# dohlee/diffab-pytorch

Hardware: AMD Instinct MI355X
Metric: CDR-residue denoise-steps/sec (K=128 patch) (higher is better)
Workload: dtype f32 (bf16x6 / fp16x3 split-precision products on the 16-bit matrix cores, fp32 accumulate; fp32-accurate, DESIGN section 4)

## Files before the change

diffab-pytorch_amd/csrc/ipa_persistent.hip:

```cpp
#include "common.h"
#include "denoiser_internal.h"
#define AT_STAMP_REALTIME 1
#include "ipa_attn_tile.h"
#include "proj_frames_h3_tile.h"
#include "rowgemm_h3_tile.h"
#include "mlp_chain_tile.h"

namespace diffab {

namespace {
constexpr size_t cmax(size_t a, size_t b) { return a > b ? a : b; }
constexpr size_t kModuleLdsBytes = cmax(cmax(ipa_attn_lds_bytes(8), static_cast<size_t>(kChainLdsBytes)),
                                        cmax(static_cast<size_t>(pjh3::PJ_LDS_BYTES), static_cast<size_t>(h3tile::lds_bytes<128>())));

struct ModuleArgs {
  float* xa;
  float* xb;
  float* proj;
  float* feat;
  const float* pair;
  const float* esc;
  const int* ctx_of_row;
  const float* R;
  const float* t;
  const char* planes;
  size_t layer_stride, pj_off, out_off, wis_off, small_off;
  unsigned long long* stamps;
  const float* emb_X;
  MlpChainSet emb, heads;
  int B, NL;
  int stagger_ticks, stagger_classes;
};
}

template <int KRES>
__global__ __launch_bounds__(512) void ipa_module_persistent_kernel(const ModuleArgs a) {
  extern __shared__ __attribute__((aligned(16))) float lds[];
  constexpr int K = KRES, NTILE = K / TI, DT = K / 128;
  static_assert(KRES == 128 || KRES == 256, "patch-resident module: K = 128 or 256");
  const int M = a.B * K;
  if (a.stagger_ticks > 0 && a.stagger_classes > 1) {
    const unsigned long long t0 = __builtin_amdgcn_s_memrealtime();
    const unsigned long long wait = static_cast<unsigned long long>((blockIdx.x >> 3) % a.stagger_classes) * a.stagger_ticks;
    while (__builtin_amdgcn_s_memrealtime() - t0 < wait) __builtin_amdgcn_s_sleep(32);
  }
  unsigned long long* pstamps = a.stamps ? a.stamps + static_cast<size_t>(a.B) * a.NL * NTILE * 64 : nullptr;
  auto pstamp = [&](int b, int l, int k) {
    if (pstamps != nullptr && threadIdx.x == 0) pstamps[(static_cast<size_t>(b) * a.NL + l) * 4 + k] = __builtin_amdgcn_s_memrealtime();
  };
#pragma unroll 1
  for (int b = blockIdx.x; b < a.B; b += gridDim.x) {
    if (a.emb_X != nullptr) {
#pragma unroll 1
      for (int dt = 0; dt < DT; ++dt) {
        int tid = threadIdx.x;
        asm volatile("" : "+v"(tid));
        chaintile::mlp_chain_tile(reinterpret_cast<__bf16*>(lds), tid, b * DT + dt, a.emb_X, 128, a.emb.c[0].planes[0], a.emb.c[0].planes[1],
                                  nullptr, a.emb.c[0].bias[0], a.emb.c[0].bias[1], nullptr, a.emb.c[0].bias_idx0, a.emb.c[0].bias_div0, 2, 128,
                                  a.xa, 128, M);
        asm volatile("s_waitcnt vmcnt(0)" ::: "memory");
        __syncthreads();
      }
    }
#pragma unroll 1
    for (int l = 0; l < a.NL; ++l) {
      const char* lp = a.planes + static_cast<size_t>(l) * a.layer_stride;
      const float* small = reinterpret_cast<const float*>(lp + a.small_off);
      const float* xin = (l & 1) ? a.xb : a.xa;
      float* xout = (l & 1) ? a.xa : a.xb;
      pstamp(b, l, 0);
#pragma unroll 1
      for (int dt = 0; dt < DT; ++dt) {
        int tid = threadIdx.x;
        asm volatile("" : "+v"(tid));
        pjh3::proj_frames_h3_tile<true, false>(reinterpret_cast<_Float16*>(lds), tid, b * DT + dt, 0, 1, xin,
                                               reinterpret_cast<const _Float16*>(lp + a.pj_off), reinterpret_cast<const float*>(lp + a.wis_off),
                                               a.R, a.t, a.proj, M);
        if (dt + 1 < DT) {
          asm volatile("s_waitcnt vmcnt(0)" ::: "memory");
          __syncthreads();
        }
      }
      asm volatile("s_waitcnt vmcnt(0)" ::: "memory");
      __syncthreads();
      pstamp(b, l, 1);
#pragma unroll 1
      for (int tile = 0; tile < NTILE; ++tile) {
        ipa_attn_tile<8, (KRES > 128), true>(lds, b, tile, static_cast<unsigned>((b * a.NL + l) * NTILE + tile), a.proj, a.pair, a.R, a.t, small,
                                             small + 512, a.feat, K / 128, a.stamps, a.esc, nullptr, nullptr, a.ctx_of_row);
        asm volatile("s_waitcnt vmcnt(0)" ::: "memory");
        __syncthreads();
      }
      pstamp(b, l, 2);
#pragma unroll 1
      for (int dt = 0; dt < DT; ++dt) {
        int tid = threadIdx.x;
        asm volatile("" : "+v"(tid));
        h3tile::rowgemm128_h3_tile<false, 128>(reinterpret_cast<_Float16*>(lds), tid, b * DT + dt, a.feat, AF,
                                               reinterpret_cast<const _Float16*>(lp + a.out_off),
                                               reinterpret_cast<const float*>(lp + a.wis_off) + ANP, small + 576, nullptr, 0, xout, 128, M, AF);
        if (dt + 1 < DT) {
          asm volatile("s_waitcnt vmcnt(0)" ::: "memory");
          __syncthreads();
        }
      }
      asm volatile("s_waitcnt vmcnt(0)" ::: "memory");
      __syncthreads();
      pstamp(b, l, 3);
    }
    if (a.emb_X != nullptr) {
      const float* xfin = (a.NL & 1) ? a.xb : a.xa;
#pragma unroll 1
      for (int hdt = 0; hdt < 3 * DT; ++hdt) {
        const int hd = hdt / DT, dt = hdt % DT;
        int tid = threadIdx.x;
        asm volatile("" : "+v"(tid));
#define HSEL(f) (hd == 0 ? a.heads.c[0].f : hd == 1 ? a.heads.c[1].f : a.heads.c[2].f)
        chaintile::mlp_chain_tile(reinterpret_cast<__bf16*>(lds), tid, b * DT + dt, xfin, 128, HSEL(planes[0]), HSEL(planes[1]), HSEL(planes[2]),
                                  HSEL(bias[0]), HSEL(bias[1]), HSEL(bias[2]), HSEL(bias_idx0), HSEL(bias_div0), 3, HSEL(n_out),
                                  hd == 0 ? a.heads.Y[0] : hd == 1 ? a.heads.Y[1] : a.heads.Y[2],
                                  hd == 0 ? a.heads.ldy[0] : hd == 1 ? a.heads.ldy[1] : a.heads.ldy[2], M);
#undef HSEL
        asm volatile("s_waitcnt vmcnt(0)" ::: "memory");
        __syncthreads();
      }
    }
  }
}

namespace {
int g_stagger_ticks = 1000, g_stagger_classes = 8;
unsigned long long* g_module_stamps = nullptr;
}
void set_module_stagger(int ticks, int classes) {
  g_stagger_ticks = ticks;
  g_stagger_classes = classes;
}
void set_module_stamps(void* p) { g_module_stamps = static_cast<unsigned long long*>(p); }

bool ipa_module_persistent_supported(const diffab_dims* d) {
  return fast_path_supported(d) && (d->K == 128 || d->K == 256) && d->NL >= 1;
}

int launch_ipa_module_persistent(const diffab_dims* d, float* xa, float* xb, const float* R, const float* t, float* ws, const void* planes,
                                 const float* pair_planes, hipStream_t st, const float* emb_X, const MlpChainSet* emb,
                                 const MlpChainSet* heads, const int* ctx_of_row, int n_ctx) {
  DIFFAB_REQUIRE(ipa_module_persistent_supported(d) && xa && xb && R && t && ws && planes && pair_planes, DIFFAB_ERR_ARG,
                 "ipa_module_persistent: unsupported operands");
  const size_t rows = static_cast<size_t>(d->B) * d->K;
  ModuleArgs a{};
  a.xa = xa;
  a.xb = xb;
  a.proj = ws;
  a.feat = ws + rows * ANP;
  a.pair = pair_planes + 64;
  a.esc = pair_row_scales(d, pair_planes, n_ctx);
  a.ctx_of_row = ctx_of_row;
  a.R = R;
  a.t = t;
  a.planes = static_cast<const char*>(planes);
  a.layer_stride = ipa_layer_planes_bytes();
  a.pj_off = ipa_layer_h3_pj_offset();
  a.out_off = ipa_layer_h3_out_offset();
  a.wis_off = ipa_layer_h3_wis_offset();
  a.small_off = ipa_layer_small_offset();
  a.stamps = g_module_stamps;
  if (emb_X != nullptr) {
    DIFFAB_REQUIRE(emb && heads && d->D == 128 && (reinterpret_cast<uintptr_t>(emb_X) & 15) == 0, DIFFAB_ERR_ARG,
                   "ipa_module_persistent: the fused MLP phases need both chain sets");
    a.emb_X = emb_X;
    a.emb = *emb;
    a.heads = *heads;
  }
  a.B = d->B;
  a.NL = d->NL;
  a.stagger_ticks = g_stagger_ticks;
  a.stagger_classes = g_stagger_classes;
  int dev = 0, ncu = 256;
  if (hipGetDevice(&dev) == hipSuccess) (void)hipDeviceGetAttribute(&ncu, hipDeviceAttributeMultiprocessorCount, dev);
  const int grid = d->B < ncu ? d->B : ncu;
#define MODULE_LAUNCH(K_)                                                                                                       \
  do {                                                                                                                            \
    DIFFAB_HIP_CHECK(hipFuncSetAttribute(reinterpret_cast<const void*>(ipa_module_persistent_kernel<K_>),                         \
                                         hipFuncAttributeMaxDynamicSharedMemorySize, static_cast<int>(kModuleLdsBytes)));        \
    timer_begin(st);                                                                                                              \
    hipLaunchKernelGGL((ipa_module_persistent_kernel<K_>), dim3(grid), dim3(512), kModuleLdsBytes, st, a);                        \
    timer_end(st);                                                                                                                \
  } while (0)
  if (d->K == 128) MODULE_LAUNCH(128);
  else MODULE_LAUNCH(256);
#undef MODULE_LAUNCH
  DIFFAB_LAUNCH_CHECK();
  return DIFFAB_OK;
}

}
```

diffab-pytorch_amd/csrc/proj_frames_h3_tile.h:

```cpp
#pragma once
#include <hip/hip_runtime.h>
#include <cstdint>

#include "rowgemm_h3_tile.h"

namespace diffab {
namespace pjh3 {
using h3tile::f16x8;
using h3tile::f32x4;
using h3tile::h3_scale;
using h3tile::split2;
#define PJH3_FENCE() asm volatile("" ::: "memory")
constexpr int PJ_NP = 1344, PJ_GQ = 768;
constexpr int PJ_B = 96, PJ_NB = PJ_NP / PJ_B, PJ_ROWS = 128;
constexpr int PJ_LD = 80;
constexpr int PJ_STAGE_ELEMS = 2 * PJ_B * 64;
constexpr int PJ_STAGE_LDS = 2 * PJ_B * PJ_LD;
constexpr int PJ_LDS_BYTES = 2 * PJ_STAGE_LDS * 2 + PJ_ROWS * 12 * 4 + PJ_ROWS * 4;
struct __attribute__((packed, aligned(4))) pj_f3 { float x, y, z; };
__device__ __forceinline__ float mul1(float a, float b) {
#pragma clang fp contract(off)
  return a * b;
}

template <bool FULL, bool SPLIT = false, bool PROJ = true>
__device__ __forceinline__ void proj_frames_h3_tile(_Float16* __restrict__ pj_lds, const int tid, const int tile_m, const int split_i,
                                                    const int split_n, const float* __restrict__ X, const _Float16* __restrict__ Wc,
                                                    const float* __restrict__ wis, const float* __restrict__ R, const float* __restrict__ t,
                                                    float* __restrict__ Y, int M, const int nb_rt = 0, const int n_rt = 0, const int ldy_rt = 0) {
  const int NB = PROJ ? PJ_NB : nb_rt, ldy = PROJ ? PJ_NP : ldy_rt, frames_from = PROJ ? PJ_GQ / PJ_B : NB;
  const int blk0 = SPLIT ? (NB * split_i) / split_n : 0;
  const int blk1 = SPLIT ? (NB * (split_i + 1)) / split_n : NB;
  float* Rt = reinterpret_cast<float*>(pj_lds + 2 * PJ_STAGE_LDS);
  float* Sx = Rt + PJ_ROWS * 12;
  const int lane = tid & 63, wv = tid >> 6;
  const int l15 = lane & 15, g = lane >> 4, rw = wv & 3, cw = wv >> 2;
  const int m0 = tile_m * PJ_ROWS;
  float* ybase = Y + static_cast<int64_t>(m0 + 32 * rw + 4 * g) * ldy + 48 * cw + 3 * l15;
  const int col0 = 48 * cw + 3 * l15;

  int st_dst[3];
#pragma unroll
  for (int i = 0; i < 3; ++i) {
    const int idx = tid + 512 * i, pl = idx / 768, rem = idx % 768;
    st_dst[i] = (pl * PJ_B + (rem >> 3)) * PJ_LD + (rem & 7) * 8;
  }
  f32x4 wreg[3];
  const int NSTAGE = 2 * blk1;
  auto load_w = [&](int stg) {
    stg = stg < NSTAGE ? stg : NSTAGE - 1;
    const _Float16* src = Wc + static_cast<size_t>(stg) * PJ_STAGE_ELEMS + tid * 8;
#pragma unroll
    for (int i = 0; i < 3; ++i) wreg[i] = *reinterpret_cast<const f32x4*>(src + 512 * 8 * i);
  };
  auto store_w = [&](int buf) {
#pragma unroll
    for (int i = 0; i < 3; ++i) *reinterpret_cast<f32x4*>(pj_lds + buf * PJ_STAGE_LDS + st_dst[i]) = wreg[i];
  };
  load_w(2 * blk0);
  f16x8 a[2][4][2];
#pragma unroll
  for (int mt = 0; mt < 2; ++mt) {
    const int row = m0 + 32 * rw + 16 * mt + l15;
    f32x4 v[4][2];
    float m = 0.0f;
#pragma unroll
    for (int q = 0; q < 4; ++q) {
      v[q][0] = v[q][1] = f32x4{0.f, 0.f, 0.f, 0.f};
      if (FULL || row < M) {
        const float* xp = X + static_cast<int64_t>(row) * 128 + 32 * q + 8 * g;
        v[q][0] = *reinterpret_cast<const f32x4*>(xp);
        v[q][1] = *reinterpret_cast<const f32x4*>(xp + 4);
      }
#pragma unroll
      for (int c = 0; c < 8; ++c) m = fmaxf(m, fabsf(v[q][c >> 2][c & 3]));
    }
    m = fmaxf(m, __shfl_xor(m, 16));
    m = fmaxf(m, __shfl_xor(m, 32));
    float s, is;
    h3_scale(m, s, is);
    if (g == 0) Sx[32 * rw + 16 * mt + l15] = is;
#pragma unroll
    for (int q = 0; q < 4; ++q)
#pragma unroll
      for (int c = 0; c < 8; ++c) {
        _Float16 h1, h2;
        split2(v[q][c >> 2][c & 3] * s, h1, h2);
        a[mt][q][0][c] = h1;
        a[mt][q][1][c] = h2;
      }
  }
  for (int idx = tid; PROJ && idx < PJ_ROWS * 12; idx += 512) {
    const int row = idx / 12, cc = idx % 12, gr = m0 + row;
    float v = 0.0f;
    if (FULL || gr < M) v = cc < 9 ? R[static_cast<int64_t>(gr) * 9 + cc] : t[static_cast<int64_t>(gr) * 3 + (cc - 9)];
    Rt[idx] = v;
  }
  PJH3_FENCE();
  store_w(0);
  load_w(2 * blk0 + 1);
  PJH3_FENCE();
  __syncthreads();

  auto epilogue_piece = [&](const f32x4 (&acc)[2][3], const pj_f3 wsc, int blk, int piece) {
    const int mt = piece >> 2, r = piece & 3;
    const int lrow = 32 * rw + 16 * mt + 4 * g + r;
    const float isx = Sx[lrow];
    const float vx = mul1(acc[mt][0][r], mul1(isx, wsc.x)), vy = mul1(acc[mt][1][r], mul1(isx, wsc.y)), vz0 = mul1(acc[mt][2][r], mul1(isx, wsc.z));
    float ox = vx, oy = vy, oz = vz0;
    if (PROJ && blk >= frames_from) {
      const f32x4* F = reinterpret_cast<const f32x4*>(Rt + lrow * 12);
      const f32x4 f0 = F[0], f1 = F[1], f2 = F[2];
      const float vz = vz0;
      ox = __builtin_fmaf(vz, f1[2], __builtin_fmaf(vy, f0[3], mul1(vx, f0[0]))) + f2[1];
      oy = __builtin_fmaf(vz, f1[3], __builtin_fmaf(vy, f1[0], mul1(vx, f0[1]))) + f2[2];
      oz = __builtin_fmaf(vz, f2[0], __builtin_fmaf(vy, f1[1], mul1(vx, f0[2]))) + f2[3];
    }
    if (FULL || m0 + lrow < M) {
      float* yp = ybase + (16 * mt + r) * ldy + PJ_B * blk;
      if constexpr (PROJ) {
        pj_f3 o{ox, oy, oz};
        *reinterpret_cast<pj_f3*>(yp) = o;
      } else {
        const int c = PJ_B * blk + col0;
        if (c < n_rt) yp[0] = ox;
        if (c + 1 < n_rt) yp[1] = oy;
        if (c + 2 < n_rt) yp[2] = oz;
      }
    }
  };
  auto run_block = [&](f32x4 (&cur)[2][3], const f32x4 (&prev)[2][3], const pj_f3 wprev, int blk) {
#pragma unroll
    for (int mt = 0; mt < 2; ++mt)
#pragma unroll
      for (int tt = 0; tt < 3; ++tt) cur[mt][tt] = f32x4{0.f, 0.f, 0.f, 0.f};
#pragma unroll
    for (int kh = 0; kh < 2; ++kh) {
      store_w(kh ^ 1);
      load_w(2 * blk + kh + 2);
      PJH3_FENCE();
      const _Float16* wl = pj_lds + kh * PJ_STAGE_LDS + (48 * cw + l15) * PJ_LD + 8 * g;
#pragma unroll
      for (int ks = 0; ks < 2; ++ks) {
        f16x8 b[3][2];
#pragma unroll
        for (int pl = 0; pl < 2; ++pl)
#pragma unroll
          for (int tt = 0; tt < 3; ++tt) b[tt][pl] = *reinterpret_cast<const f16x8*>(wl + (pl * PJ_B + 16 * tt) * PJ_LD + 32 * ks);
#pragma unroll
        for (int term = 0; term < 3; ++term) {
          const int pa = term == 0 ? 1 : 0, pb = term == 1 ? 1 : 0;
#pragma unroll
          for (int mt = 0; mt < 2; ++mt)
#pragma unroll
            for (int tt = 0; tt < 3; ++tt)
              cur[mt][tt] = __builtin_amdgcn_mfma_f32_16x16x32_f16(a[mt][2 * kh + ks][pa], b[tt][pb], cur[mt][tt], 0, 0, 0);
          if (kh == 0 && blk > blk0) {
            epilogue_piece(prev, wprev, blk - 1, 4 * ks + term);
            if (term == 2) epilogue_piece(prev, wprev, blk - 1, 4 * ks + 3);
            __builtin_amdgcn_sched_barrier(0);
          }
        }
      }
      __syncthreads();
    }
  };
  auto wsc_of = [&](int blk) { return *reinterpret_cast<const pj_f3*>(wis + PJ_B * blk + col0); };
  f32x4 accA[2][3], accB[2][3];
  pj_f3 wA = wsc_of(blk0), wB = wA;
  int blk = blk0;
  for (; blk + 1 < blk1; blk += 2) {
    run_block(accA, accB, wB, blk);
    wB = wsc_of(blk + 1);
    run_block(accB, accA, wA, blk + 1);
    if (blk + 2 < blk1) wA = wsc_of(blk + 2);
  }
  if ((SPLIT || !PROJ) && blk < blk1) {
    run_block(accA, accB, wB, blk);
#pragma unroll
    for (int piece = 0; piece < 8; ++piece) epilogue_piece(accA, wA, blk, piece);
  } else {
#pragma unroll
    for (int piece = 0; piece < 8; ++piece) epilogue_piece(accB, wB, blk1 - 1, piece);
  }
}
#undef PJH3_FENCE
}
}
```

diffab-pytorch_amd/csrc/rowgemm_h3_tile.h:

```cpp
#pragma once
#include <hip/hip_runtime.h>

namespace diffab {
namespace h3tile {
typedef float f32x4 __attribute__((ext_vector_type(4)));
typedef _Float16 f16x8 __attribute__((ext_vector_type(8)));
typedef _Float16 f16x4 __attribute__((ext_vector_type(4)));
typedef float f32x16 __attribute__((ext_vector_type(16)));
constexpr int BK = 32;
constexpr int PART_CHUNKS = 2;

__device__ __forceinline__ int h3_off(int row, int slot) { return row * BK + 8 * (slot ^ ((row >> 2) & 3)); }
__device__ __forceinline__ void h3_scale(float m, float& s, float& is) {
  const int e = static_cast<int>((__float_as_uint(m) >> 23) & 255u);
  const bool ok = e >= 8 && e < 231;
  s = ok ? __uint_as_float(static_cast<unsigned>(127 + 7 + 127 - e) << 23) : 1.0f;
  is = ok ? __uint_as_float(static_cast<unsigned>(e - 7) << 23) : 1.0f;
}
__device__ __forceinline__ void split2(float x, _Float16& h1, _Float16& h2) {
  h1 = static_cast<_Float16>(x);
  h2 = static_cast<_Float16>(x - static_cast<float>(h1));
}
template <int ROWS>
constexpr int lds_bytes() { return 2 * 2 * (128 + ROWS) * BK * 2 + 2 * ROWS * 4; }

template <bool RELU, int ROWS, bool PARTIAL = false>
__device__ __forceinline__ void rowgemm128_h3_tile(_Float16* h3_lds, int tid, int tile_m, const float* __restrict__ X, int ldx,
                                                   const _Float16* __restrict__ Wc, const float* __restrict__ wis, const float* __restrict__ bias,
                                                   const int64_t* __restrict__ bias_idx, int bias_div, float* __restrict__ Y, int ldy, int M, int Kd,
                                                   int c_begin = 0, float* __restrict__ part_out = nullptr) {
#define H3TILE_FENCE() asm volatile("" ::: "memory")
  constexpr int T = ROWS * 4, NRW = ROWS / 32;
  _Float16* Ws = h3_lds;
  _Float16* As = h3_lds + 2 * 2 * 128 * BK;
  float* Sx = reinterpret_cast<float*>(As + 2 * 2 * ROWS * BK);
  const int lane = tid & 63, wv = tid >> 6;
  const int l31 = lane & 31, hk = lane >> 5, rw = wv % NRW, cw = wv / NRW;
  const int m0 = tile_m * ROWS;
  const int nchunk = PARTIAL ? min(Kd / BK, c_begin + PART_CHUNKS) : Kd / BK;
  constexpr int WP = 1024 / T;
  int w_dst[WP];
#pragma unroll
  for (int i = 0; i < WP; ++i) {
    const int idx = tid + T * i, p = idx / 512, row = (idx % 512) >> 2, part = idx & 3;
    w_dst[i] = (p * 128) * BK + h3_off(row, part);
  }
  f32x4 wreg[2][WP];
  auto load_w = [&](int slot, int ch) {
    ch = ch < nchunk ? ch : nchunk - 1;
    const _Float16* src = Wc + static_cast<size_t>(ch) * (2 * 128 * BK) + tid * 8;
#pragma unroll
    for (int i = 0; i < WP; ++i) wreg[slot][i] = *reinterpret_cast<const f32x4*>(src + T * 8 * i);
  };
  auto store_w = [&](int slot, int buf) {
#pragma unroll
    for (int i = 0; i < WP; ++i) *reinterpret_cast<f32x4*>(Ws + buf * (2 * 128 * BK) + w_dst[i]) = wreg[slot][i];
  };
  const int xa_row = tid >> 3, xa_part = tid & 7;
  const float* xsrc[2];
  int x_dst[2];
#pragma unroll
  for (int j = 0; j < 2; ++j) {
    const int lrow = xa_row + (ROWS / 2) * j;
    int row = m0 + lrow;
    row = row < M ? row : M - 1;
    xsrc[j] = X + static_cast<int64_t>(row) * ldx + 4 * xa_part;
    x_dst[j] = h3_off(lrow, xa_part >> 1) + 4 * (xa_part & 1);
  }
  f32x4 xreg[4][2];
  auto load_x = [&](int slot, int ch) {
    ch = ch < nchunk ? ch : nchunk - 1;
#pragma unroll
    for (int j = 0; j < 2; ++j) xreg[slot][j] = *reinterpret_cast<const f32x4*>(xsrc[j] + ch * BK);
  };
  float sx_cur[2];
  auto pair_scale = [&](int slot_a, int slot_b, int pp) {
#pragma unroll
    for (int j = 0; j < 2; ++j) {
      const f32x4 va = xreg[slot_a][j], vb = xreg[slot_b][j];
      float m = fmaxf(fmaxf(fmaxf(fabsf(va[0]), fabsf(va[1])), fmaxf(fabsf(va[2]), fabsf(va[3]))),
                      fmaxf(fmaxf(fabsf(vb[0]), fabsf(vb[1])), fmaxf(fabsf(vb[2]), fabsf(vb[3]))));
      m = fmaxf(m, __shfl_xor(m, 1));
      m = fmaxf(m, __shfl_xor(m, 2));
      m = fmaxf(m, __shfl_xor(m, 4));
      float is;
      h3_scale(m, sx_cur[j], is);
      if (xa_part == 0) Sx[pp * ROWS + xa_row + (ROWS / 2) * j] = is;
    }
  };
  auto store_x = [&](int slot, int buf) {
#pragma unroll
    for (int j = 0; j < 2; ++j) {
      const f32x4 v = xreg[slot][j];
      f16x4 h1, h2;
#pragma unroll
      for (int c = 0; c < 4; ++c) {
        _Float16 a, b;
        split2(v[c] * sx_cur[j], a, b);
        h1[c] = a; h2[c] = b;
      }
      _Float16* dst = As + buf * (2 * ROWS * BK) + x_dst[j];
      *reinterpret_cast<f16x4*>(dst) = h1;
      *reinterpret_cast<f16x4*>(dst + ROWS * BK) = h2;
    }
  };
  f32x16 acc[2], tot[2];
#pragma unroll
  for (int tt = 0; tt < 2; ++tt)
#pragma unroll
    for (int r = 0; r < 16; ++r) acc[tt][r] = tot[tt][r] = 0.f;

#pragma unroll
  for (int c = 0; c < 4; ++c) load_x(c, c_begin + c);
  load_w(0, c_begin);
  load_w(1, c_begin + 1);
  H3TILE_FENCE();
  store_w(0, 0);
  pair_scale(0, 1, 0);
  store_x(0, 0);
  load_w(0, c_begin + 2);
  load_x(0, c_begin + 4);
  H3TILE_FENCE();
  __syncthreads();
  const int fx = (l31 >> 2) & 3;
  const int a_off = (32 * rw + l31) * BK, w_off = (64 * cw + l31) * BK;
  for (int ch0 = c_begin; ch0 < nchunk; ch0 += 4) {
#pragma unroll
    for (int u = 0; u < 4; ++u) {
      const int ch = ch0 + u, buf = u & 1;
      if (ch >= nchunk) break;
      const _Float16* al = As + buf * (2 * ROWS * BK) + a_off;
      const _Float16* wl = Ws + buf * (2 * 128 * BK) + w_off;
#pragma unroll
      for (int ks = 0; ks < 2; ++ks) {
        const int so = 8 * ((2 * ks + hk) ^ fx);
        f16x8 a[2], b[2][2];
#pragma unroll
        for (int p = 0; p < 2; ++p) {
          a[p] = *reinterpret_cast<const f16x8*>(al + (p * ROWS) * BK + so);
#pragma unroll
          for (int tt = 0; tt < 2; ++tt) b[tt][p] = *reinterpret_cast<const f16x8*>(wl + (p * 128 + 32 * tt) * BK + so);
        }
#pragma unroll
        for (int tt = 0; tt < 2; ++tt) acc[tt] = __builtin_amdgcn_mfma_f32_32x32x16_f16(a[1], b[tt][0], acc[tt], 0, 0, 0);
#pragma unroll
        for (int tt = 0; tt < 2; ++tt) acc[tt] = __builtin_amdgcn_mfma_f32_32x32x16_f16(a[0], b[tt][1], acc[tt], 0, 0, 0);
#pragma unroll
        for (int tt = 0; tt < 2; ++tt) acc[tt] = __builtin_amdgcn_mfma_f32_32x32x16_f16(a[0], b[tt][0], acc[tt], 0, 0, 0);
      }
      store_w((u + 1) & 1, buf ^ 1);
      if (u & 1) pair_scale((u + 1) & 3, (u + 2) & 3, ((u + 1) >> 1) & 1);
      store_x((u + 1) & 3, buf ^ 1);
      load_w((u + 1) & 1, ch + 3);
      load_x((u + 1) & 3, ch + 5);
      H3TILE_FENCE();
      if (u & 1) {
        f32x4 sx[4];
#pragma unroll
        for (int g = 0; g < 4; ++g) sx[g] = *reinterpret_cast<const f32x4*>(Sx + (u >> 1) * ROWS + 32 * rw + 8 * g + 4 * hk);
#pragma unroll
        for (int tt = 0; tt < 2; ++tt)
#pragma unroll
          for (int r = 0; r < 16; ++r) {
            tot[tt][r] = __builtin_fmaf(acc[tt][r], sx[r >> 2][r & 3], tot[tt][r]);
            acc[tt][r] = 0.f;
          }
      }
      __syncthreads();
    }
  }
  if (PARTIAL) {
#pragma unroll
    for (int tt = 0; tt < 2; ++tt)
#pragma unroll
      for (int r = 0; r < 16; ++r)
        part_out[(32 * rw + (r & 3) + 8 * (r >> 2) + 4 * hk) * 128 + 64 * cw + 32 * tt + l31] = tot[tt][r];
    return;
  }
  const bool table = bias_idx != nullptr || bias_div > 0;
#pragma unroll
  for (int tt = 0; tt < 2; ++tt) {
    const int col = 64 * cw + 32 * tt + l31;
    const float wi = wis[col];
    float bv = (bias && !table) ? bias[col] : 0.0f;
#pragma unroll
    for (int r = 0; r < 16; ++r) {
      const int row = m0 + 32 * rw + (r & 3) + 8 * (r >> 2) + 4 * hk;
      if (row >= M) continue;
      if (table) {
        const int64_t bi = bias_idx ? bias_idx[row] : row / bias_div;
        bv = bias[bi * 128 + col];
      }
      float o = __builtin_fmaf(tot[tt][r], wi, bv);
      if (RELU) o = fmaxf(o, 0.f);
      Y[static_cast<int64_t>(row) * ldy + col] = o;
    }
  }
#undef H3TILE_FENCE
}
}
}
```

Measured before the change: 13.25 million.

## Keep the residue activation tile resident in LDS across IPA layers for K=128

For K=128 patches, the persistent module kernel loads the x activation tile into a dedicated LDS region once at layer 0. The output rowgemm writes its result back into that region, and the next layer's projection reads x from LDS instead of global memory. Global writes of x happen only on the last layer. This removes one global store and one global load of the activations per layer, but it relies on the attention and other phases never overwriting that LDS region. The padded row stride of 132 adds LDS footprint.

```diff
diff --git a/diffab-pytorch_amd/csrc/ipa_persistent.hip b/diffab-pytorch_amd/csrc/ipa_persistent.hip
--- a/diffab-pytorch_amd/csrc/ipa_persistent.hip
+++ b/diffab-pytorch_amd/csrc/ipa_persistent.hip
@@ -12,6 +12,10 @@
 constexpr size_t cmax(size_t a, size_t b) { return a > b ? a : b; }
 constexpr size_t kModuleLdsBytes = cmax(cmax(ipa_attn_lds_bytes(8), static_cast<size_t>(kChainLdsBytes)),
                                         cmax(static_cast<size_t>(pjh3::PJ_LDS_BYTES), static_cast<size_t>(h3tile::lds_bytes<128>())));
+constexpr size_t kXImageOffset = cmax(static_cast<size_t>(pjh3::PJ_LDS_BYTES), static_cast<size_t>(h3tile::lds_bytes<128>())) / 4;
+static_assert(kXImageOffset * 4 + h3tile::y_lds_bytes<128>() <= kModuleLdsBytes, "module LDS: no room for the x image of the dense phases");
+static_assert(kModuleLdsBytes <= 160 * 1024, "module LDS: one work-group per CU within gfx950's 160 KiB");
+static_assert(kXImageOffset % 4 == 0, "x image: 16-byte aligned rows");
 
 struct ModuleArgs {
   float* xa;
@@ -73,9 +77,25 @@
       for (int dt = 0; dt < DT; ++dt) {
         int tid = threadIdx.x;
         asm volatile("" : "+v"(tid));
-        pjh3::proj_frames_h3_tile<true, false>(reinterpret_cast<_Float16*>(lds), tid, b * DT + dt, 0, 1, xin,
-                                               reinterpret_cast<const _Float16*>(lp + a.pj_off), reinterpret_cast<const float*>(lp + a.wis_off),
-                                               a.R, a.t, a.proj, M);
+        if (KRES == 128) {
+          if (l == 0) {
+            float* xl = lds + kXImageOffset;
+            for (int i = tid; i < 128 * 32; i += 512) {
+              const int row = i >> 5, c4 = 4 * (i & 31);
+              *reinterpret_cast<float4*>(xl + row * h3tile::Y_LDS_LD + c4) =
+                  *reinterpret_cast<const float4*>(xin + (static_cast<int64_t>(b) * 128 + row) * 128 + c4);
+            }
+            __syncthreads();
+          }
+          pjh3::proj_frames_h3_tile<true, false, true, true>(reinterpret_cast<_Float16*>(lds), tid, b, 0, 1, nullptr,
+                                                             reinterpret_cast<const _Float16*>(lp + a.pj_off),
+                                                             reinterpret_cast<const float*>(lp + a.wis_off), a.R, a.t, a.proj, M, 0, 0, 0,
+                                                             lds + kXImageOffset);
+        } else {
+          pjh3::proj_frames_h3_tile<true, false>(reinterpret_cast<_Float16*>(lds), tid, b * DT + dt, 0, 1, xin,
+                                                 reinterpret_cast<const _Float16*>(lp + a.pj_off), reinterpret_cast<const float*>(lp + a.wis_off),
+                                                 a.R, a.t, a.proj, M);
+        }
         if (dt + 1 < DT) {
           asm volatile("s_waitcnt vmcnt(0)" ::: "memory");
           __syncthreads();
@@ -96,9 +116,15 @@
       for (int dt = 0; dt < DT; ++dt) {
         int tid = threadIdx.x;
         asm volatile("" : "+v"(tid));
-        h3tile::rowgemm128_h3_tile<false, 128>(reinterpret_cast<_Float16*>(lds), tid, b * DT + dt, a.feat, AF,
-                                               reinterpret_cast<const _Float16*>(lp + a.out_off),
-                                               reinterpret_cast<const float*>(lp + a.wis_off) + ANP, small + 576, nullptr, 0, xout, 128, M, AF);
+        if (KRES == 128)
+          h3tile::rowgemm128_h3_tile<false, 128, false, true>(reinterpret_cast<_Float16*>(lds), tid, b, a.feat, AF,
+                                                              reinterpret_cast<const _Float16*>(lp + a.out_off),
+                                                              reinterpret_cast<const float*>(lp + a.wis_off) + ANP, small + 576, nullptr, 0,
+                                                              l + 1 == a.NL ? xout : nullptr, 128, M, AF, 0, nullptr, lds + kXImageOffset);
+        else
+          h3tile::rowgemm128_h3_tile<false, 128>(reinterpret_cast<_Float16*>(lds), tid, b * DT + dt, a.feat, AF,
+                                                 reinterpret_cast<const _Float16*>(lp + a.out_off),
+                                                 reinterpret_cast<const float*>(lp + a.wis_off) + ANP, small + 576, nullptr, 0, xout, 128, M, AF);
         if (dt + 1 < DT) {
           asm volatile("s_waitcnt vmcnt(0)" ::: "memory");
           __syncthreads();
diff --git a/diffab-pytorch_amd/csrc/proj_frames_h3_tile.h b/diffab-pytorch_amd/csrc/proj_frames_h3_tile.h
--- a/diffab-pytorch_amd/csrc/proj_frames_h3_tile.h
+++ b/diffab-pytorch_amd/csrc/proj_frames_h3_tile.h
@@ -23,11 +23,12 @@
   return a * b;
 }
 
-template <bool FULL, bool SPLIT = false, bool PROJ = true>
+template <bool FULL, bool SPLIT = false, bool PROJ = true, bool X_LDS = false>
 __device__ __forceinline__ void proj_frames_h3_tile(_Float16* __restrict__ pj_lds, const int tid, const int tile_m, const int split_i,
                                                     const int split_n, const float* __restrict__ X, const _Float16* __restrict__ Wc,
                                                     const float* __restrict__ wis, const float* __restrict__ R, const float* __restrict__ t,
-                                                    float* __restrict__ Y, int M, const int nb_rt = 0, const int n_rt = 0, const int ldy_rt = 0) {
+                                                    float* __restrict__ Y, int M, const int nb_rt = 0, const int n_rt = 0, const int ldy_rt = 0,
+                                                    const float* __restrict__ x_lds = nullptr) {
   const int NB = PROJ ? PJ_NB : nb_rt, ldy = PROJ ? PJ_NP : ldy_rt, frames_from = PROJ ? PJ_GQ / PJ_B : NB;
   const int blk0 = SPLIT ? (NB * split_i) / split_n : 0;
   const int blk1 = SPLIT ? (NB * (split_i + 1)) / split_n : NB;
@@ -68,7 +69,8 @@
     for (int q = 0; q < 4; ++q) {
       v[q][0] = v[q][1] = f32x4{0.f, 0.f, 0.f, 0.f};
       if (FULL || row < M) {
-        const float* xp = X + static_cast<int64_t>(row) * 128 + 32 * q + 8 * g;
+        const float* xp = X_LDS ? x_lds + (row - m0) * h3tile::Y_LDS_LD + 32 * q + 8 * g
+                                : X + static_cast<int64_t>(row) * 128 + 32 * q + 8 * g;
         v[q][0] = *reinterpret_cast<const f32x4*>(xp);
         v[q][1] = *reinterpret_cast<const f32x4*>(xp + 4);
       }
diff --git a/diffab-pytorch_amd/csrc/rowgemm_h3_tile.h b/diffab-pytorch_amd/csrc/rowgemm_h3_tile.h
--- a/diffab-pytorch_amd/csrc/rowgemm_h3_tile.h
+++ b/diffab-pytorch_amd/csrc/rowgemm_h3_tile.h
@@ -24,11 +24,15 @@
 template <int ROWS>
 constexpr int lds_bytes() { return 2 * 2 * (128 + ROWS) * BK * 2 + 2 * ROWS * 4; }
 
-template <bool RELU, int ROWS, bool PARTIAL = false>
+constexpr int Y_LDS_LD = 132;
+template <int ROWS>
+constexpr int y_lds_bytes() { return ROWS * Y_LDS_LD * 4; }
+
+template <bool RELU, int ROWS, bool PARTIAL = false, bool Y_LDS = false>
 __device__ __forceinline__ void rowgemm128_h3_tile(_Float16* h3_lds, int tid, int tile_m, const float* __restrict__ X, int ldx,
                                                    const _Float16* __restrict__ Wc, const float* __restrict__ wis, const float* __restrict__ bias,
                                                    const int64_t* __restrict__ bias_idx, int bias_div, float* __restrict__ Y, int ldy, int M, int Kd,
-                                                   int c_begin = 0, float* __restrict__ part_out = nullptr) {
+                                                   int c_begin = 0, float* __restrict__ part_out = nullptr, float* __restrict__ y_lds = nullptr) {
 #define H3TILE_FENCE() asm volatile("" ::: "memory")
   constexpr int T = ROWS * 4, NRW = ROWS / 32;
   _Float16* Ws = h3_lds;
@@ -178,6 +182,7 @@
     return;
   }
   const bool table = bias_idx != nullptr || bias_div > 0;
+  const bool y_global = !Y_LDS || Y != nullptr;
 #pragma unroll
   for (int tt = 0; tt < 2; ++tt) {
     const int col = 64 * cw + 32 * tt + l31;
@@ -193,7 +198,8 @@
       }
       float o = __builtin_fmaf(tot[tt][r], wi, bv);
       if (RELU) o = fmaxf(o, 0.f);
-      Y[static_cast<int64_t>(row) * ldy + col] = o;
+      if (Y_LDS) y_lds[(row - m0) * Y_LDS_LD + col] = o;
+      if (y_global) Y[static_cast<int64_t>(row) * ldy + col] = o;
     }
   }
 #undef H3TILE_FENCE
```

New measurement: 13.45 million (median of 6 runs). 1.5% higher.
